# pythoncrazy/jimm

Hardware: AMD Instinct MI355X
Metric: images/sec (whole node) ViT-B/16@224 train (higher is better)
Workload: dtype bf16; 1 GPU; model=ViT-B/16@224, global_batch=1024, img_size=224, parallelism=dp1

## Files before the change

jimm_amd/csrc/gemm.hip:

```cpp

#include <torch/extension.h>
#include <ATen/hip/HIPContext.h>

#include "common.h"

namespace {

typedef short bf16x8_t __attribute__((ext_vector_type(8)));
typedef float f32x4_t __attribute__((ext_vector_type(4)));

#define MFMA16(A, B, C) __builtin_amdgcn_mfma_f32_16x16x32_bf16(A, B, C, 0, 0, 0)

constexpr int BM = 128, BN = 128, BK = 64;
constexpr int PITCH = BK + 8;



__device__ __forceinline__ void stage_tile_glds(const bf16* __restrict__ gsrc, int64_t ldg,
                                                short* lds_base, int tid) {
  const int wave = tid / WAVE;
  const int lane = tid % WAVE;
#pragma unroll
  for (int round = 0; round < 4; ++round) {
    const int off = round * 4096 + wave * 1024 + lane * 16;
    const int row = off >> 7;
    const int chunk = (off >> 4) & 7;
    const int src_chunk = chunk ^ (row & 7);
    const bf16* g = gsrc + (int64_t)row * ldg + src_chunk * 8;
    typedef const __attribute__((address_space(1))) unsigned int* gp_t;
    typedef __attribute__((address_space(3))) unsigned int* lp_t;
    __builtin_amdgcn_global_load_lds((gp_t)(const void*)g,
                                     (lp_t)(void*)(reinterpret_cast<char*>(lds_base) + round * 4096 + wave * 1024),
                                     16, 0, 0);
  }
}

__device__ __forceinline__ bf16x8_t lds_read_frag(const short* base, int row, int chunk) {
  const int byte = (row << 7) + ((chunk ^ (row & 7)) << 4);
  return *reinterpret_cast<const bf16x8_t*>(reinterpret_cast<const char*>(base) + byte);
}

template <int ACT, bool HAS_BIAS, bool HAS_RES, bool SAVE_PRE>
__global__ __launch_bounds__(256) void gemm_nt_fast_kernel(
    const bf16* __restrict__ X, const bf16* __restrict__ W, const float* __restrict__ bias,
    const bf16* __restrict__ res, bf16* __restrict__ Y, bf16* __restrict__ Z,
    int M, int N, int K) {
  extern __shared__ __attribute__((aligned(16))) char smem[];
  short* smem_s = reinterpret_cast<short*>(smem);
  auto xs = [&](int buf) { return smem_s + buf * 8192; };
  auto ws = [&](int buf) { return smem_s + 16384 + buf * 8192; };

  const int tid = threadIdx.x;
  const int lane = tid % WAVE;
  const int wave = tid / WAVE;
  const int lo = lane & 15, hi = lane >> 4;

  const int mt = M / BM, nt = N / BN;
  const int nwg = mt * nt;
  int wg = blockIdx.x;
  {
    const int q = nwg / 8, r = nwg % 8;
    const int xcd = wg % 8, idx = wg / 8;
    wg = (xcd < r ? xcd * (q + 1) : r * (q + 1) + (xcd - r) * q) + idx;
  }
  const int m0 = (wg / nt) * BM;
  const int n0 = (wg % nt) * BN;
  const int wm = (wave >> 1) * 64, wn = (wave & 1) * 64;

  f32x4_t acc[4][4] = {};

  stage_tile_glds(X + (int64_t)m0 * K, K, xs(0), tid);
  stage_tile_glds(W + (int64_t)n0 * K, K, ws(0), tid);
  __syncthreads();

  const int nk = K / BK;
  for (int kt = 0; kt < nk; ++kt) {
    const int buf = kt & 1;
    if (kt + 1 < nk) {
      stage_tile_glds(X + (int64_t)m0 * K + (kt + 1) * BK, K, xs(buf ^ 1), tid);
      stage_tile_glds(W + (int64_t)n0 * K + (kt + 1) * BK, K, ws(buf ^ 1), tid);
    }
#pragma unroll
    for (int ks = 0; ks < 2; ++ks) {
      bf16x8_t xa[4], wb[4];
#pragma unroll
      for (int mi = 0; mi < 4; ++mi) xa[mi] = lds_read_frag(xs(buf), wm + 16 * mi + lo, 4 * ks + hi);
#pragma unroll
      for (int ni = 0; ni < 4; ++ni) wb[ni] = lds_read_frag(ws(buf), wn + 16 * ni + lo, 4 * ks + hi);
#pragma unroll
      for (int mi = 0; mi < 4; ++mi)
#pragma unroll
        for (int ni = 0; ni < 4; ++ni) acc[mi][ni] = MFMA16(xa[mi], wb[ni], acc[mi][ni]);
    }
    __syncthreads();
  }

#pragma unroll
  for (int mi = 0; mi < 4; ++mi) {
#pragma unroll
    for (int r = 0; r < 4; ++r) {
      const int m = m0 + wm + 16 * mi + hi * 4 + r;
#pragma unroll
      for (int ni = 0; ni < 4; ++ni) {
        const int n = n0 + wn + 16 * ni + lo;
        float vpre = acc[mi][ni][r];
        if (HAS_BIAS) vpre += bias[n];
        if (SAVE_PRE) Z[(int64_t)m * N + n] = f2bf(vpre);
        float vy = act_fwd(vpre, ACT);
        if (HAS_RES) vy += bf2f(res[(int64_t)m * N + n]);
        Y[(int64_t)m * N + n] = f2bf(vy);
      }
    }
  }
}


template <int ACT, bool HAS_BIAS, bool HAS_RES, bool SAVE_PRE>
__global__ __launch_bounds__(256) void gemm_nt_kernel(
    const bf16* __restrict__ X, const bf16* __restrict__ W, const float* __restrict__ bias,
    const bf16* __restrict__ res, bf16* __restrict__ Y, bf16* __restrict__ Z,
    int M, int N, int K) {
  extern __shared__ __attribute__((aligned(16))) char smem[];
  short* xs = reinterpret_cast<short*>(smem);
  short* ws = xs + 2 * BM * PITCH;

  const int tid = threadIdx.x;
  const int wave = tid / WAVE;
  const int lane = tid % WAVE;
  const int lo = lane & 15, hi = lane >> 4;

  const int m0 = blockIdx.x * BM;
  const int n0 = blockIdx.y * BN;
  const int wm = (wave >> 1) * 64;
  const int wn = (wave & 1) * 64;

  f32x4_t acc[4][4] = {};

  auto stage = [&](int buf, int k0) {
    short* xd = xs + buf * BM * PITCH;
    short* wd = ws + buf * BN * PITCH;
    const int row = tid / 2;
    const int c0 = (tid & 1) * 32;
#pragma unroll
    for (int h = 0; h < 2; ++h) {
      const int cc = c0 + h * 16;
      if (m0 + row < M) {
        *reinterpret_cast<bf16x8_t*>(xd + row * PITCH + cc) =
            *reinterpret_cast<const bf16x8_t*>(X + (int64_t)(m0 + row) * K + k0 + cc);
        *reinterpret_cast<bf16x8_t*>(xd + row * PITCH + cc + 8) =
            *reinterpret_cast<const bf16x8_t*>(X + (int64_t)(m0 + row) * K + k0 + cc + 8);
      } else {
        for (int i = 0; i < 16; ++i) xd[row * PITCH + cc + i] = 0;
      }
      if (n0 + row < N) {
        *reinterpret_cast<bf16x8_t*>(wd + row * PITCH + cc) =
            *reinterpret_cast<const bf16x8_t*>(W + (int64_t)(n0 + row) * K + k0 + cc);
        *reinterpret_cast<bf16x8_t*>(wd + row * PITCH + cc + 8) =
            *reinterpret_cast<const bf16x8_t*>(W + (int64_t)(n0 + row) * K + k0 + cc + 8);
      } else {
        for (int i = 0; i < 16; ++i) wd[row * PITCH + cc + i] = 0;
      }
    }
  };

  stage(0, 0);
  __syncthreads();

  const int nk = K / BK;
  for (int kt = 0; kt < nk; ++kt) {
    const int buf = kt & 1;
    if (kt + 1 < nk) stage(buf ^ 1, (kt + 1) * BK);
    short* xd = xs + buf * BM * PITCH;
    short* wd = ws + buf * BN * PITCH;
#pragma unroll
    for (int ks = 0; ks < 2; ++ks) {
      bf16x8_t xa[4], wb[4];
#pragma unroll
      for (int mi = 0; mi < 4; ++mi)
        xa[mi] = *reinterpret_cast<const bf16x8_t*>(xd + (wm + 16 * mi + lo) * PITCH + 32 * ks + hi * 8);
#pragma unroll
      for (int ni = 0; ni < 4; ++ni)
        wb[ni] = *reinterpret_cast<const bf16x8_t*>(wd + (wn + 16 * ni + lo) * PITCH + 32 * ks + hi * 8);
#pragma unroll
      for (int mi = 0; mi < 4; ++mi)
#pragma unroll
        for (int ni = 0; ni < 4; ++ni)
          acc[mi][ni] = MFMA16(xa[mi], wb[ni], acc[mi][ni]);
    }
    __syncthreads();
  }

#pragma unroll
  for (int mi = 0; mi < 4; ++mi) {
#pragma unroll
    for (int r = 0; r < 4; ++r) {
      const int m = m0 + wm + 16 * mi + hi * 4 + r;
      if (m >= M) continue;
#pragma unroll
      for (int ni = 0; ni < 4; ++ni) {
        const int n = n0 + wn + 16 * ni + lo;
        if (n >= N) continue;
        float vpre = acc[mi][ni][r];
        if (HAS_BIAS) vpre += bias[n];
        if (SAVE_PRE) Z[(int64_t)m * N + n] = f2bf(vpre);
        float vy = act_fwd(vpre, ACT);
        if (HAS_RES) vy += bf2f(res[(int64_t)m * N + n]);
        Y[(int64_t)m * N + n] = f2bf(vy);
      }
    }
  }
}

}

bool gemm256_supported(int64_t M, int64_t N, int64_t K);
void gemm_nt_256(torch::Tensor x, torch::Tensor w, c10::optional<torch::Tensor> bias_f32,
                 std::string act, c10::optional<torch::Tensor> residual, torch::Tensor y,
                 c10::optional<torch::Tensor> z);
bool gemm8p_supported(int64_t M, int64_t N, int64_t K);
void gemm_nt_8p(torch::Tensor x, torch::Tensor w, c10::optional<torch::Tensor> bias_f32,
                std::string act, c10::optional<torch::Tensor> residual, torch::Tensor y,
                c10::optional<torch::Tensor> z);

static int gemm_tile_mode() {
  const char* env = getenv("JIMM_AMD_GEMM_TILE");
  if (!env) return 0;
  return atoi(env);
}

bool gemm_supported(int64_t M, int64_t N, int64_t K, std::string dtype) {
  if (dtype != "torch.bfloat16") return false;
  if (K % BK != 0) return false;
  const char* env = getenv("JIMM_AMD_GEMM");
  if (env && std::string(env) == "blas") return false;
  return true;
}

std::vector<torch::Tensor> linear_fwd(torch::Tensor x, torch::Tensor w,
                                      c10::optional<torch::Tensor> bias, std::string act,
                                      c10::optional<torch::Tensor> residual, bool save_z) {
  TORCH_CHECK(x.is_cuda() && x.is_contiguous() && w.is_contiguous());
  TORCH_CHECK(x.scalar_type() == torch::kBFloat16 && w.scalar_type() == torch::kBFloat16);
  const int M = x.size(0), K = x.size(1), N = w.size(0);
  TORCH_CHECK(w.size(1) == K && K % BK == 0);
  auto y = torch::empty({M, N}, x.options());
  torch::Tensor z;
  if (save_z) z = torch::empty({M, N}, x.options());
  c10::optional<torch::Tensor> bf;
  if (bias) bf = bias->contiguous().to(torch::kFloat32);
  int act_code = ACT_NONE;
  if (act == "gelu") act_code = ACT_GELU;
  else if (act == "gelu_tanh") act_code = ACT_GELU_TANH;
  else if (act == "quickgelu") act_code = ACT_QUICKGELU;
  else TORCH_CHECK(act.empty(), "unknown act ", act);

  const int tile_mode = gemm_tile_mode();
  if (tile_mode == 0 && gemm8p_supported(M, N, K)) {
    c10::optional<torch::Tensor> zopt;
    if (save_z) zopt = z;
    gemm_nt_8p(x, w, bf, act, residual, y, zopt);
    if (save_z) return {y, z};
    return {y, torch::Tensor()};
  }
  if (tile_mode != 128 && gemm256_supported(M, N, K)) {
    c10::optional<torch::Tensor> zopt;
    if (save_z) zopt = z;
    gemm_nt_256(x, w, bf, act, residual, y, zopt);
    if (save_z) return {y, z};
    return {y, torch::Tensor()};
  }

  auto stream = at::hip::getCurrentHIPStream();
  const bf16* resp = residual ? reinterpret_cast<const bf16*>(residual->data_ptr()) : nullptr;
  const float* biasp = bf ? bf->data_ptr<float>() : nullptr;
  bf16* zp = save_z ? reinterpret_cast<bf16*>(z.data_ptr()) : nullptr;
  const bool fast = (M % BM == 0) && (N % BN == 0);

#define LAUNCH(ACTC, HB, HR, SP)                                                          \
  do {                                                                                    \
    if (fast) {                                                                           \
      hipLaunchKernelGGL((gemm_nt_fast_kernel<ACTC, HB, HR, SP>),                         \
                         dim3((M / BM) * (N / BN)), dim3(256), 4 * 8192 * sizeof(short),  \
                         stream, reinterpret_cast<const bf16*>(x.data_ptr()),             \
                         reinterpret_cast<const bf16*>(w.data_ptr()), biasp, resp,        \
                         reinterpret_cast<bf16*>(y.data_ptr()), zp, M, N, K);             \
    } else {                                                                              \
      hipLaunchKernelGGL((gemm_nt_kernel<ACTC, HB, HR, SP>),                              \
                         dim3((M + BM - 1) / BM, (N + BN - 1) / BN), dim3(256),           \
                         2 * (BM + BN) * PITCH * sizeof(short), stream,                   \
                         reinterpret_cast<const bf16*>(x.data_ptr()),                     \
                         reinterpret_cast<const bf16*>(w.data_ptr()), biasp, resp,        \
                         reinterpret_cast<bf16*>(y.data_ptr()), zp, M, N, K);             \
    }                                                                                     \
  } while (0)
#define DISPATCH_ACT(HB, HR, SP)                                                          \
  switch (act_code) {                                                                     \
    case ACT_NONE: LAUNCH(ACT_NONE, HB, HR, SP); break;                                   \
    case ACT_GELU: LAUNCH(ACT_GELU, HB, HR, SP); break;                                   \
    case ACT_GELU_TANH: LAUNCH(ACT_GELU_TANH, HB, HR, SP); break;                         \
    case ACT_QUICKGELU: LAUNCH(ACT_QUICKGELU, HB, HR, SP); break;                         \
  }
  const bool hb = bias.has_value(), hr = residual.has_value();
  if (hb && hr && save_z) DISPATCH_ACT(true, true, true)
  else if (hb && hr) DISPATCH_ACT(true, true, false)
  else if (hb && save_z) DISPATCH_ACT(true, false, true)
  else if (hb) DISPATCH_ACT(true, false, false)
  else if (hr && save_z) DISPATCH_ACT(false, true, true)
  else if (hr) DISPATCH_ACT(false, true, false)
  else if (save_z) DISPATCH_ACT(false, false, true)
  else DISPATCH_ACT(false, false, false)
#undef DISPATCH_ACT
#undef LAUNCH
  if (save_z) return {y, z};
  return {y, torch::Tensor()};
}
```

jimm_amd/csrc/gemm8p.hip:

```cpp

#include <torch/extension.h>
#include <hip/hip_fp8.h>
#include <ATen/hip/HIPContext.h>

#include "common.h"

namespace {

typedef short bf16x8_t __attribute__((ext_vector_type(8)));
typedef float f32x4_t __attribute__((ext_vector_type(4)));

#define MFMA16(A, B, C) __builtin_amdgcn_mfma_f32_16x16x32_bf16(A, B, C, 0, 0, 0)

constexpr int BM = 256, BN = 256, BK = 64;
constexpr int NTHREADS = 512;
constexpr int HALF_BYTES = 128 * BK * 2;

__device__ __forceinline__ void raw_barrier() {
  asm volatile("s_barrier" ::: "memory");
}

template <bool MGUARD>
__device__ __forceinline__ const bf16* stage_base(const bf16* __restrict__ gsrc,
                                                  int64_t ldg, int row0, int rows_total,
                                                  int round, int tid) {
  const int off = round * 8192 + tid * 16;
  const int row = off >> 7;
  const int chunk = ((off >> 4) & 7) ^ (row & 7);
  int grow = row0 + row;
  if (MGUARD) grow = grow < rows_total ? grow : rows_total - 1;
  return gsrc + (int64_t)grow * ldg + chunk * 8;
}

__device__ __forceinline__ void glds16(const bf16* g, char* lds_dst) {
  typedef const __attribute__((address_space(1))) unsigned int* gp_t;
  typedef __attribute__((address_space(3))) unsigned int* lp_t;
  __builtin_amdgcn_global_load_lds((gp_t)(const void*)g, (lp_t)(void*)lds_dst, 16, 0, 0);
}

__device__ __forceinline__ bf16x8_t lds_frag8p(const char* base, int byte_off) {
  return *reinterpret_cast<const bf16x8_t*>(base + byte_off);
}

__device__ __forceinline__ int frag_off(int row, int chunk) {
  return (row << 7) + ((chunk ^ (row & 7)) << 4);
}

template <int ACT, bool HAS_BIAS, bool HAS_RES, bool SAVE_PRE, bool MGUARD, bool GRADM = false,
          bool FP8O = false>
__global__ __launch_bounds__(NTHREADS, 2) void gemm_nt_8p_kernel(
    const bf16* __restrict__ X, const bf16* __restrict__ W, const float* __restrict__ bias,
    const bf16* __restrict__ res, bf16* __restrict__ Y, bf16* __restrict__ Z,
    int M, int N, int K, unsigned char* __restrict__ Y8 = nullptr,
    const float* __restrict__ scale8 = nullptr,
    unsigned int* __restrict__ amax_bits = nullptr) {
  extern __shared__ __attribute__((aligned(16))) char smem[];
  auto As = [&](int buf, int h) { return smem + (buf * 2 + h) * HALF_BYTES; };
  auto Bs = [&](int slot, int h) {
    return smem + 4 * HALF_BYTES + (slot * 2 + h) * HALF_BYTES;
  };

  const int tid = threadIdx.x;
  const int lane = tid % WAVE;
  const int wave = tid / WAVE;
  const int lo = lane & 15, hi = lane >> 4;

  const int mt = MGUARD ? (M + BM - 1) / BM : M / BM;
  const int nt = N / BN;
  const int nwg = mt * nt;
  int wg = blockIdx.x;
  {
    const int q = nwg / 8, r = nwg % 8;
    const int xcd = wg % 8, idx = wg / 8;
    wg = (xcd < r ? xcd * (q + 1) : r * (q + 1) + (xcd - r) * q) + idx;
  }
  const int m0 = (wg / nt) * BM;
  const int n0 = (wg % nt) * BN;
  const int wm = (wave >> 2);
  const int wn = (wave & 3);

  f32x4_t acc[2][4][4] = {};

  const int nk = K / BK;
  const bf16* asrc[2][2];
  const bf16* bsrc[2][2];
#pragma unroll
  for (int h = 0; h < 2; ++h)
#pragma unroll
    for (int r = 0; r < 2; ++r) {
      asrc[h][r] = stage_base<MGUARD>(X, K, m0 + h * 128, M, r, tid);
      bsrc[h][r] = stage_base<false>(W + (int64_t)n0 * K, K, h * 128, N, r, tid);
    }
  const int ldst = tid * 16;
  auto stageA = [&](int kt, int h) {
    char* img = As(kt & 1, h);
    glds16(asrc[h][0] + (int64_t)kt * BK, img + ldst);
    glds16(asrc[h][1] + (int64_t)kt * BK, img + 8192 + ldst);
  };
  auto stageB = [&](int kt, int slot, int h) {
    char* img = Bs(slot, h);
    glds16(bsrc[h][0] + (int64_t)kt * BK, img + ldst);
    glds16(bsrc[h][1] + (int64_t)kt * BK, img + 8192 + ldst);
  };

  int offA[2][4], offB[2][4];
#pragma unroll
  for (int kh = 0; kh < 2; ++kh) {
#pragma unroll
    for (int mi = 0; mi < 4; ++mi)
      offA[kh][mi] = frag_off(wm * 64 + 16 * mi + lo, 4 * kh + hi);
#pragma unroll
    for (int ni = 0; ni < 4; ++ni)
      offB[kh][ni] = frag_off((wn & 1) * 64 + 16 * ni + lo, 4 * kh + hi);
  }
  const int bh = wn >> 1;

  stageB(0, 0, 0);
  stageB(0, 0, 1);
  stageA(0, 0);
  stageA(0, 1);
  asm volatile("s_waitcnt vmcnt(2)" ::: "memory");
  raw_barrier();

  int slot = 0, slot1 = nk > 1 ? 1 : 0;
  for (int t = 0; t < nk; ++t) {
    const int buf = t & 1;
    const char* a0i = As(buf, 0);
    const char* a1i = As(buf, 1);
    const char* bi = Bs(slot, bh);
    const bool more = t + 1 < nk;
#pragma unroll
    for (int kh = 0; kh < 2; ++kh) {
      bf16x8_t xa[4], wb[4];
#pragma unroll
      for (int mi = 0; mi < 4; ++mi) xa[mi] = lds_frag8p(a0i, offA[kh][mi]);
#pragma unroll
      for (int ni = 0; ni < 4; ++ni) wb[ni] = lds_frag8p(bi, offB[kh][ni]);
      if (more) {
        if (kh == 0) stageB(t + 1, slot1, 0);
        else stageA(t + 1, 0);
      }
      if (kh == 0) {
        if (t == nk - 1) asm volatile("s_waitcnt vmcnt(0)" ::: "memory");
        else asm volatile("s_waitcnt vmcnt(2)" ::: "memory");
      } else {
        asm volatile("s_waitcnt vmcnt(4)" ::: "memory");
      }
      raw_barrier();
      __builtin_amdgcn_s_setprio(1);
#pragma unroll
      for (int mi = 0; mi < 4; ++mi)
#pragma unroll
        for (int ni = 0; ni < 4; ++ni)
          acc[0][mi][ni] = MFMA16(xa[mi], wb[ni], acc[0][mi][ni]);
      __builtin_amdgcn_s_setprio(0);

#pragma unroll
      for (int mi = 0; mi < 4; ++mi) xa[mi] = lds_frag8p(a1i, offA[kh][mi]);
      if (more) {
        if (kh == 0) stageB(t + 1, slot1, 1);
        else stageA(t + 1, 1);
      }
      if (kh == 0) asm volatile("s_waitcnt vmcnt(4)" ::: "memory");
      else asm volatile("s_waitcnt vmcnt(2)" ::: "memory");
      raw_barrier();
      __builtin_amdgcn_s_setprio(1);
#pragma unroll
      for (int mi = 0; mi < 4; ++mi)
#pragma unroll
        for (int ni = 0; ni < 4; ++ni)
          acc[1][mi][ni] = MFMA16(xa[mi], wb[ni], acc[1][mi][ni]);
      __builtin_amdgcn_s_setprio(0);
    }
    slot = slot1;
    slot1 = slot1 + 1 == 3 ? 0 : slot1 + 1;
  }

  float rs8 = 1.f, tmax = 0.f;
  if (FP8O) rs8 = 1.f / scale8[0];
#pragma unroll
  for (int pr = 0; pr < 2; ++pr) {
#pragma unroll
    for (int mi = 0; mi < 4; ++mi) {
#pragma unroll
      for (int r = 0; r < 4; ++r) {
        const int m = m0 + pr * 128 + wm * 64 + 16 * mi + hi * 4 + r;
        if (MGUARD && m >= M) continue;
#pragma unroll
        for (int ni = 0; ni < 4; ++ni) {
          const int n = n0 + wn * 64 + 16 * ni + lo;
          float vpre = acc[pr][mi][ni][r];
          if (HAS_BIAS) vpre += bias[n];
          if (SAVE_PRE) Z[(int64_t)m * N + n] = f2bf(vpre);
          float vy;
          if (GRADM) {
            vy = vpre * act_grad(bf2f(res[(int64_t)m * N + n]), ACT);
          } else {
            vy = act_fwd(vpre, ACT);
            if (HAS_RES) vy += bf2f(res[(int64_t)m * N + n]);
          }
          Y[(int64_t)m * N + n] = f2bf(vy);
          if (FP8O) {
            tmax = fmaxf(tmax, fabsf(vy));
            Y8[(int64_t)m * N + n] = cvt_e4m3(vy * rs8);
          }
        }
      }
    }
  }
  if (FP8O) {
    tmax = wave_reduce_max(tmax);
    if (lane == 0) atomicMax(amax_bits, __float_as_uint(tmax));
  }
}

}

bool gemm8p_supported(int64_t M, int64_t N, int64_t K) {
  return M >= 1 && (N % BN == 0) && (K % BK == 0) && K >= 2 * BK;
}

torch::Tensor gemm_nt_8p_gradact(torch::Tensor dy, torch::Tensor wt, torch::Tensor z,
                                 std::string act) {
  const int M = dy.size(0), K = dy.size(1), N = wt.size(0);
  TORCH_CHECK(dy.is_contiguous() && wt.is_contiguous() && z.is_contiguous());
  TORCH_CHECK(wt.size(1) == K && z.size(0) == M && z.size(1) == N);
  TORCH_CHECK(gemm8p_supported(M, N, K));
  int act_code = ACT_NONE;
  if (act == "gelu") act_code = ACT_GELU;
  else if (act == "gelu_tanh") act_code = ACT_GELU_TANH;
  else if (act == "quickgelu") act_code = ACT_QUICKGELU;
  else TORCH_CHECK(false, "gradact needs an activation, got ", act);
  auto y = torch::empty({M, N}, dy.options());
  auto stream = at::hip::getCurrentHIPStream();
  const size_t shmem = 10 * HALF_BYTES;
  const bool mguard = (M % BM) != 0;
  const int mt = (M + BM - 1) / BM;
#define LAUNCH_GRAD(ACTC, MG)                                                              \
  do {                                                                                     \
    auto kfn = gemm_nt_8p_kernel<ACTC, false, true, false, MG, true>;                      \
    static bool attr_g_##ACTC##MG = [&] {                                                  \
      hipFuncSetAttribute(reinterpret_cast<const void*>(kfn),                              \
                          hipFuncAttributeMaxDynamicSharedMemorySize, (int)shmem);         \
      return true;                                                                         \
    }();                                                                                   \
    (void)attr_g_##ACTC##MG;                                                               \
    hipLaunchKernelGGL(kfn, dim3(mt * (N / BN)), dim3(NTHREADS), shmem, stream,            \
                       reinterpret_cast<const bf16*>(dy.data_ptr()),                       \
                       reinterpret_cast<const bf16*>(wt.data_ptr()), nullptr,              \
                       reinterpret_cast<const bf16*>(z.data_ptr()),                        \
                       reinterpret_cast<bf16*>(y.data_ptr()), nullptr, M, N, K,            \
                       nullptr, nullptr, nullptr);                                         \
  } while (0)
#define DG(ACTC)                                                                           \
  do {                                                                                     \
    if (mguard) LAUNCH_GRAD(ACTC, true);                                                   \
    else LAUNCH_GRAD(ACTC, false);                                                         \
  } while (0)
  switch (act_code) {
    case ACT_GELU: DG(ACT_GELU); break;
    case ACT_GELU_TANH: DG(ACT_GELU_TANH); break;
    case ACT_QUICKGELU: DG(ACT_QUICKGELU); break;
  }
#undef DG
#undef LAUNCH_GRAD
  return y;
}

std::vector<torch::Tensor> gemm_nt_8p_gradact_fp8(torch::Tensor dy, torch::Tensor wt,
                                                  torch::Tensor z, std::string act,
                                                  torch::Tensor scale8, torch::Tensor amax) {
  const int M = dy.size(0), K = dy.size(1), N = wt.size(0);
  TORCH_CHECK(dy.is_contiguous() && wt.is_contiguous() && z.is_contiguous());
  TORCH_CHECK(wt.size(1) == K && z.size(0) == M && z.size(1) == N);
  TORCH_CHECK(gemm8p_supported(M, N, K));
  int act_code = ACT_NONE;
  if (act == "gelu") act_code = ACT_GELU;
  else if (act == "gelu_tanh") act_code = ACT_GELU_TANH;
  else if (act == "quickgelu") act_code = ACT_QUICKGELU;
  else TORCH_CHECK(false, "gradact needs an activation, got ", act);
  auto y = torch::empty({M, N}, dy.options());
  auto y8 = torch::empty({M, N}, dy.options().dtype(torch::kUInt8));
  auto stream = at::hip::getCurrentHIPStream();
  const size_t shmem = 10 * HALF_BYTES;
  const bool mguard = (M % BM) != 0;
  const int mt = (M + BM - 1) / BM;
#define LAUNCH_GRAD8(ACTC, MG)                                                             \
  do {                                                                                     \
    auto kfn = gemm_nt_8p_kernel<ACTC, false, true, false, MG, true, true>;                \
    static bool attr_g8_##ACTC##MG = [&] {                                                 \
      hipFuncSetAttribute(reinterpret_cast<const void*>(kfn),                              \
                          hipFuncAttributeMaxDynamicSharedMemorySize, (int)shmem);         \
      return true;                                                                         \
    }();                                                                                   \
    (void)attr_g8_##ACTC##MG;                                                              \
    hipLaunchKernelGGL(kfn, dim3(mt * (N / BN)), dim3(NTHREADS), shmem, stream,            \
                       reinterpret_cast<const bf16*>(dy.data_ptr()),                       \
                       reinterpret_cast<const bf16*>(wt.data_ptr()), nullptr,              \
                       reinterpret_cast<const bf16*>(z.data_ptr()),                        \
                       reinterpret_cast<bf16*>(y.data_ptr()), nullptr, M, N, K,            \
                       y8.data_ptr<unsigned char>(), scale8.data_ptr<float>(),             \
                       reinterpret_cast<unsigned int*>(amax.data_ptr()));                  \
  } while (0)
#define DG8(ACTC)                                                                          \
  do {                                                                                     \
    if (mguard) LAUNCH_GRAD8(ACTC, true);                                                  \
    else LAUNCH_GRAD8(ACTC, false);                                                        \
  } while (0)
  switch (act_code) {
    case ACT_GELU: DG8(ACT_GELU); break;
    case ACT_GELU_TANH: DG8(ACT_GELU_TANH); break;
    case ACT_QUICKGELU: DG8(ACT_QUICKGELU); break;
  }
#undef DG8
#undef LAUNCH_GRAD8
  return {y, y8};
}

void gemm_nt_8p(torch::Tensor x, torch::Tensor w, c10::optional<torch::Tensor> bias_f32,
                std::string act, c10::optional<torch::Tensor> residual, torch::Tensor y,
                c10::optional<torch::Tensor> z) {
  const int M = x.size(0), K = x.size(1), N = w.size(0);
  TORCH_CHECK(gemm8p_supported(M, N, K));
  int act_code = ACT_NONE;
  if (act == "gelu") act_code = ACT_GELU;
  else if (act == "gelu_tanh") act_code = ACT_GELU_TANH;
  else if (act == "quickgelu") act_code = ACT_QUICKGELU;
  else TORCH_CHECK(act.empty(), "unknown act ", act);
  auto stream = at::hip::getCurrentHIPStream();
  const bf16* resp = residual ? reinterpret_cast<const bf16*>(residual->data_ptr()) : nullptr;
  const float* biasp = bias_f32 ? bias_f32->data_ptr<float>() : nullptr;
  bf16* zp = z ? reinterpret_cast<bf16*>(z->data_ptr()) : nullptr;
  const size_t shmem = 10 * HALF_BYTES;
  const bool mguard = (M % BM) != 0;
  const int mt = (M + BM - 1) / BM;

#define LAUNCH8P(ACTC, HB, HR, SP, MG)                                                     \
  do {                                                                                     \
    auto kfn = gemm_nt_8p_kernel<ACTC, HB, HR, SP, MG>;                                    \
    static bool attr_set_##ACTC##HB##HR##SP##MG = [&] {                                    \
      hipFuncSetAttribute(reinterpret_cast<const void*>(kfn),                              \
                          hipFuncAttributeMaxDynamicSharedMemorySize, (int)shmem);         \
      return true;                                                                         \
    }();                                                                                   \
    (void)attr_set_##ACTC##HB##HR##SP##MG;                                                 \
    hipLaunchKernelGGL(kfn, dim3(mt * (N / BN)), dim3(NTHREADS), shmem, stream,            \
                       reinterpret_cast<const bf16*>(x.data_ptr()),                        \
                       reinterpret_cast<const bf16*>(w.data_ptr()), biasp, resp,           \
                       reinterpret_cast<bf16*>(y.data_ptr()), zp, M, N, K,                 \
                       nullptr, nullptr, nullptr);                                         \
  } while (0)
#define DISPATCH_MG(ACTC, HB, HR, SP)                                                      \
  do {                                                                                     \
    if (mguard) LAUNCH8P(ACTC, HB, HR, SP, true);                                          \
    else LAUNCH8P(ACTC, HB, HR, SP, false);                                                \
  } while (0)
#define DISPATCH_ACT8P(HB, HR, SP)                                                         \
  switch (act_code) {                                                                      \
    case ACT_NONE: DISPATCH_MG(ACT_NONE, HB, HR, SP); break;                               \
    case ACT_GELU: DISPATCH_MG(ACT_GELU, HB, HR, SP); break;                               \
    case ACT_GELU_TANH: DISPATCH_MG(ACT_GELU_TANH, HB, HR, SP); break;                     \
    case ACT_QUICKGELU: DISPATCH_MG(ACT_QUICKGELU, HB, HR, SP); break;                     \
  }
  const bool hb = bias_f32.has_value(), hr = residual.has_value(), sp = z.has_value();
  if (hb && hr && sp) DISPATCH_ACT8P(true, true, true)
  else if (hb && hr) DISPATCH_ACT8P(true, true, false)
  else if (hb && sp) DISPATCH_ACT8P(true, false, true)
  else if (hb) DISPATCH_ACT8P(true, false, false)
  else if (hr && sp) DISPATCH_ACT8P(false, true, true)
  else if (hr) DISPATCH_ACT8P(false, true, false)
  else if (sp) DISPATCH_ACT8P(false, false, true)
  else DISPATCH_ACT8P(false, false, false)
#undef DISPATCH_ACT8P
#undef DISPATCH_MG
#undef LAUNCH8P
}
```

Before: 5808 images/sec.

## Transpose MFMA operands and permute W rows for vectorized GEMM epilogue stores

Swaps the MFMA operand order so each lane holds 16 contiguous output columns per row, with a matching row permutation when staging the W tile so those columns line up. The epilogue then uses 16-byte vector loads and stores for bias, residual, Z, Y and the FP8 output in place of scalar per-element accesses. It also drops the per-call conversion of the bias to fp32 on the 8p path by reading bf16 bias directly. The cost is extra alignment checks and clones, and the permuted layout makes correctness more subtle.

```diff
diff --git a/jimm_amd/csrc/gemm.hip b/jimm_amd/csrc/gemm.hip
--- a/jimm_amd/csrc/gemm.hip
+++ b/jimm_amd/csrc/gemm.hip
@@ -218,7 +218,7 @@
                  std::string act, c10::optional<torch::Tensor> residual, torch::Tensor y,
                  c10::optional<torch::Tensor> z);
 bool gemm8p_supported(int64_t M, int64_t N, int64_t K);
-void gemm_nt_8p(torch::Tensor x, torch::Tensor w, c10::optional<torch::Tensor> bias_f32,
+void gemm_nt_8p(torch::Tensor x, torch::Tensor w, c10::optional<torch::Tensor> bias,
                 std::string act, c10::optional<torch::Tensor> residual, torch::Tensor y,
                 c10::optional<torch::Tensor> z);
 
@@ -246,8 +246,6 @@
   auto y = torch::empty({M, N}, x.options());
   torch::Tensor z;
   if (save_z) z = torch::empty({M, N}, x.options());
-  c10::optional<torch::Tensor> bf;
-  if (bias) bf = bias->contiguous().to(torch::kFloat32);
   int act_code = ACT_NONE;
   if (act == "gelu") act_code = ACT_GELU;
   else if (act == "gelu_tanh") act_code = ACT_GELU_TANH;
@@ -258,10 +256,14 @@
   if (tile_mode == 0 && gemm8p_supported(M, N, K)) {
     c10::optional<torch::Tensor> zopt;
     if (save_z) zopt = z;
-    gemm_nt_8p(x, w, bf, act, residual, y, zopt);
+    c10::optional<torch::Tensor> b8 = bias;
+    if (bias && bias->scalar_type() != torch::kBFloat16) b8 = bias->to(torch::kFloat32);
+    gemm_nt_8p(x, w, b8, act, residual, y, zopt);
     if (save_z) return {y, z};
     return {y, torch::Tensor()};
   }
+  c10::optional<torch::Tensor> bf;
+  if (bias) bf = bias->contiguous().to(torch::kFloat32);
   if (tile_mode != 128 && gemm256_supported(M, N, K)) {
     c10::optional<torch::Tensor> zopt;
     if (save_z) zopt = z;
diff --git a/jimm_amd/csrc/gemm8p.hip b/jimm_amd/csrc/gemm8p.hip
--- a/jimm_amd/csrc/gemm8p.hip
+++ b/jimm_amd/csrc/gemm8p.hip
@@ -20,14 +20,16 @@
   asm volatile("s_barrier" ::: "memory");
 }
 
-template <bool MGUARD>
+template <bool MGUARD, bool PERM = false>
 __device__ __forceinline__ const bf16* stage_base(const bf16* __restrict__ gsrc,
                                                   int64_t ldg, int row0, int rows_total,
                                                   int round, int tid) {
   const int off = round * 8192 + tid * 16;
   const int row = off >> 7;
   const int chunk = ((off >> 4) & 7) ^ (row & 7);
-  int grow = row0 + row;
+  int srow = row;
+  if (PERM) srow = (row & 64) | ((row & 12) << 2) | ((row >> 2) & 12) | (row & 3);
+  int grow = row0 + srow;
   if (MGUARD) grow = grow < rows_total ? grow : rows_total - 1;
   return gsrc + (int64_t)grow * ldg + chunk * 8;
 }
@@ -49,8 +51,8 @@
 template <int ACT, bool HAS_BIAS, bool HAS_RES, bool SAVE_PRE, bool MGUARD, bool GRADM = false,
           bool FP8O = false>
 __global__ __launch_bounds__(NTHREADS, 2) void gemm_nt_8p_kernel(
-    const bf16* __restrict__ X, const bf16* __restrict__ W, const float* __restrict__ bias,
-    const bf16* __restrict__ res, bf16* __restrict__ Y, bf16* __restrict__ Z,
+    const bf16* __restrict__ X, const bf16* __restrict__ W, const void* __restrict__ bias,
+    int bias_is_f32, const bf16* __restrict__ res, bf16* __restrict__ Y, bf16* __restrict__ Z,
     int M, int N, int K, unsigned char* __restrict__ Y8 = nullptr,
     const float* __restrict__ scale8 = nullptr,
     unsigned int* __restrict__ amax_bits = nullptr) {
@@ -89,7 +91,7 @@
 #pragma unroll
     for (int r = 0; r < 2; ++r) {
       asrc[h][r] = stage_base<MGUARD>(X, K, m0 + h * 128, M, r, tid);
-      bsrc[h][r] = stage_base<false>(W + (int64_t)n0 * K, K, h * 128, N, r, tid);
+      bsrc[h][r] = stage_base<false, true>(W + (int64_t)n0 * K, K, h * 128, N, r, tid);
     }
   const int ldst = tid * 16;
   auto stageA = [&](int kt, int h) {
@@ -152,7 +154,7 @@
       for (int mi = 0; mi < 4; ++mi)
 #pragma unroll
         for (int ni = 0; ni < 4; ++ni)
-          acc[0][mi][ni] = MFMA16(xa[mi], wb[ni], acc[0][mi][ni]);
+          acc[0][mi][ni] = MFMA16(wb[ni], xa[mi], acc[0][mi][ni]);
       __builtin_amdgcn_s_setprio(0);
 
 #pragma unroll
@@ -169,42 +171,86 @@
       for (int mi = 0; mi < 4; ++mi)
 #pragma unroll
         for (int ni = 0; ni < 4; ++ni)
-          acc[1][mi][ni] = MFMA16(xa[mi], wb[ni], acc[1][mi][ni]);
+          acc[1][mi][ni] = MFMA16(wb[ni], xa[mi], acc[1][mi][ni]);
       __builtin_amdgcn_s_setprio(0);
     }
     slot = slot1;
     slot1 = slot1 + 1 == 3 ? 0 : slot1 + 1;
   }
 
+  const int nb = n0 + wn * 64 + hi * 16;
+  float bv[16];
+  if (HAS_BIAS) {
+    if (bias_is_f32) {
+      const float* bp = reinterpret_cast<const float*>(bias) + nb;
+#pragma unroll
+      for (int q = 0; q < 4; ++q) {
+        float t[4];
+        vload_f32<4>(bp + 4 * q, t);
+#pragma unroll
+        for (int j = 0; j < 4; ++j) bv[4 * q + j] = t[j];
+      }
+    } else {
+      const bf16* bp = reinterpret_cast<const bf16*>(bias) + nb;
+#pragma unroll
+      for (int q = 0; q < 2; ++q) {
+        float t[8];
+        vload_f32<8>(bp + 8 * q, t);
+#pragma unroll
+        for (int j = 0; j < 8; ++j) bv[8 * q + j] = t[j];
+      }
+    }
+  }
   float rs8 = 1.f, tmax = 0.f;
   if (FP8O) rs8 = 1.f / scale8[0];
 #pragma unroll
   for (int pr = 0; pr < 2; ++pr) {
 #pragma unroll
     for (int mi = 0; mi < 4; ++mi) {
-#pragma unroll
-      for (int r = 0; r < 4; ++r) {
-        const int m = m0 + pr * 128 + wm * 64 + 16 * mi + hi * 4 + r;
-        if (MGUARD && m >= M) continue;
-#pragma unroll
-        for (int ni = 0; ni < 4; ++ni) {
-          const int n = n0 + wn * 64 + 16 * ni + lo;
+      const int m = m0 + pr * 128 + wm * 64 + 16 * mi + lo;
+      if (MGUARD && m >= M) continue;
+      const int64_t o = (int64_t)m * N + nb;
+      float rv[2][8];
+      if (HAS_RES || GRADM) {
+        vload_f32<8>(res + o, rv[0]);
+        vload_f32<8>(res + o + 8, rv[1]);
+      }
+      float vz[2][8], vo[2][8];
+#pragma unroll
+      for (int ni = 0; ni < 4; ++ni) {
+#pragma unroll
+        for (int r = 0; r < 4; ++r) {
+          const int j = 4 * ni + r;
           float vpre = acc[pr][mi][ni][r];
-          if (HAS_BIAS) vpre += bias[n];
-          if (SAVE_PRE) Z[(int64_t)m * N + n] = f2bf(vpre);
+          if (HAS_BIAS) vpre += bv[j];
+          vz[j >> 3][j & 7] = vpre;
           float vy;
           if (GRADM) {
-            vy = vpre * act_grad(bf2f(res[(int64_t)m * N + n]), ACT);
+            vy = vpre * act_grad(rv[j >> 3][j & 7], ACT);
           } else {
             vy = act_fwd(vpre, ACT);
-            if (HAS_RES) vy += bf2f(res[(int64_t)m * N + n]);
+            if (HAS_RES) vy += rv[j >> 3][j & 7];
           }
-          Y[(int64_t)m * N + n] = f2bf(vy);
-          if (FP8O) {
-            tmax = fmaxf(tmax, fabsf(vy));
-            Y8[(int64_t)m * N + n] = cvt_e4m3(vy * rs8);
-          }
+          vo[j >> 3][j & 7] = vy;
         }
+      }
+      if (SAVE_PRE) {
+        vstore_f32<8>(Z + o, vz[0]);
+        vstore_f32<8>(Z + o + 8, vz[1]);
+      }
+      vstore_f32<8>(Y + o, vo[0]);
+      vstore_f32<8>(Y + o + 8, vo[1]);
+      if (FP8O) {
+        unsigned int pk[4];
+#pragma unroll
+        for (int q = 0; q < 4; ++q) {
+          const float* v4 = &vo[q >> 1][(q & 1) * 4];
+#pragma unroll
+          for (int j = 0; j < 4; ++j) tmax = fmaxf(tmax, fabsf(v4[j]));
+          pk[q] = (unsigned int)cvt2_e4m3(v4[0] * rs8, v4[1] * rs8) |
+                  ((unsigned int)cvt2_e4m3(v4[2] * rs8, v4[3] * rs8) << 16);
+        }
+        *reinterpret_cast<uint4*>(Y8 + o) = make_uint4(pk[0], pk[1], pk[2], pk[3]);
       }
     }
   }
@@ -218,6 +264,12 @@
 
 bool gemm8p_supported(int64_t M, int64_t N, int64_t K) {
   return M >= 1 && (N % BN == 0) && (K % BK == 0) && K >= 2 * BK;
+}
+
+static torch::Tensor aligned16(const torch::Tensor& t) {
+  auto c = t.contiguous();
+  if (reinterpret_cast<uintptr_t>(c.data_ptr()) % 16 != 0) c = c.clone();
+  return c;
 }
 
 torch::Tensor gemm_nt_8p_gradact(torch::Tensor dy, torch::Tensor wt, torch::Tensor z,
@@ -226,6 +278,7 @@
   TORCH_CHECK(dy.is_contiguous() && wt.is_contiguous() && z.is_contiguous());
   TORCH_CHECK(wt.size(1) == K && z.size(0) == M && z.size(1) == N);
   TORCH_CHECK(gemm8p_supported(M, N, K));
+  z = aligned16(z);
   int act_code = ACT_NONE;
   if (act == "gelu") act_code = ACT_GELU;
   else if (act == "gelu_tanh") act_code = ACT_GELU_TANH;
@@ -247,7 +300,7 @@
     (void)attr_g_##ACTC##MG;                                                               \
     hipLaunchKernelGGL(kfn, dim3(mt * (N / BN)), dim3(NTHREADS), shmem, stream,            \
                        reinterpret_cast<const bf16*>(dy.data_ptr()),                       \
-                       reinterpret_cast<const bf16*>(wt.data_ptr()), nullptr,              \
+                       reinterpret_cast<const bf16*>(wt.data_ptr()), nullptr, 0,           \
                        reinterpret_cast<const bf16*>(z.data_ptr()),                        \
                        reinterpret_cast<bf16*>(y.data_ptr()), nullptr, M, N, K,            \
                        nullptr, nullptr, nullptr);                                         \
@@ -274,6 +327,7 @@
   TORCH_CHECK(dy.is_contiguous() && wt.is_contiguous() && z.is_contiguous());
   TORCH_CHECK(wt.size(1) == K && z.size(0) == M && z.size(1) == N);
   TORCH_CHECK(gemm8p_supported(M, N, K));
+  z = aligned16(z);
   int act_code = ACT_NONE;
   if (act == "gelu") act_code = ACT_GELU;
   else if (act == "gelu_tanh") act_code = ACT_GELU_TANH;
@@ -296,7 +350,7 @@
     (void)attr_g8_##ACTC##MG;                                                              \
     hipLaunchKernelGGL(kfn, dim3(mt * (N / BN)), dim3(NTHREADS), shmem, stream,            \
                        reinterpret_cast<const bf16*>(dy.data_ptr()),                       \
-                       reinterpret_cast<const bf16*>(wt.data_ptr()), nullptr,              \
+                       reinterpret_cast<const bf16*>(wt.data_ptr()), nullptr, 0,           \
                        reinterpret_cast<const bf16*>(z.data_ptr()),                        \
                        reinterpret_cast<bf16*>(y.data_ptr()), nullptr, M, N, K,            \
                        y8.data_ptr<unsigned char>(), scale8.data_ptr<float>(),             \
@@ -317,11 +371,24 @@
   return {y, y8};
 }
 
-void gemm_nt_8p(torch::Tensor x, torch::Tensor w, c10::optional<torch::Tensor> bias_f32,
+void gemm_nt_8p(torch::Tensor x, torch::Tensor w, c10::optional<torch::Tensor> bias,
                 std::string act, c10::optional<torch::Tensor> residual, torch::Tensor y,
                 c10::optional<torch::Tensor> z) {
   const int M = x.size(0), K = x.size(1), N = w.size(0);
   TORCH_CHECK(gemm8p_supported(M, N, K));
+  if (bias) {
+    TORCH_CHECK(bias->scalar_type() == torch::kBFloat16 ||
+                    bias->scalar_type() == torch::kFloat32,
+                "gemm_nt_8p: bias must be bf16 or fp32");
+    TORCH_CHECK(bias->numel() == N);
+    bias = aligned16(*bias);
+  }
+  if (residual) {
+    TORCH_CHECK(residual->scalar_type() == torch::kBFloat16 && residual->numel() == (int64_t)M * N);
+    residual = aligned16(*residual);
+  }
+  TORCH_CHECK(reinterpret_cast<uintptr_t>(y.data_ptr()) % 16 == 0 &&
+              (!z || reinterpret_cast<uintptr_t>(z->data_ptr()) % 16 == 0));
   int act_code = ACT_NONE;
   if (act == "gelu") act_code = ACT_GELU;
   else if (act == "gelu_tanh") act_code = ACT_GELU_TANH;
@@ -329,7 +396,8 @@
   else TORCH_CHECK(act.empty(), "unknown act ", act);
   auto stream = at::hip::getCurrentHIPStream();
   const bf16* resp = residual ? reinterpret_cast<const bf16*>(residual->data_ptr()) : nullptr;
-  const float* biasp = bias_f32 ? bias_f32->data_ptr<float>() : nullptr;
+  const void* biasp = bias ? bias->data_ptr() : nullptr;
+  const int bias_f32 = bias && bias->scalar_type() == torch::kFloat32;
   bf16* zp = z ? reinterpret_cast<bf16*>(z->data_ptr()) : nullptr;
   const size_t shmem = 10 * HALF_BYTES;
   const bool mguard = (M % BM) != 0;
@@ -346,7 +414,7 @@
     (void)attr_set_##ACTC##HB##HR##SP##MG;                                                 \
     hipLaunchKernelGGL(kfn, dim3(mt * (N / BN)), dim3(NTHREADS), shmem, stream,            \
                        reinterpret_cast<const bf16*>(x.data_ptr()),                        \
-                       reinterpret_cast<const bf16*>(w.data_ptr()), biasp, resp,           \
+                       reinterpret_cast<const bf16*>(w.data_ptr()), biasp, bias_f32, resp, \
                        reinterpret_cast<bf16*>(y.data_ptr()), zp, M, N, K,                 \
                        nullptr, nullptr, nullptr);                                         \
   } while (0)
@@ -362,7 +430,7 @@
     case ACT_GELU_TANH: DISPATCH_MG(ACT_GELU_TANH, HB, HR, SP); break;                     \
     case ACT_QUICKGELU: DISPATCH_MG(ACT_QUICKGELU, HB, HR, SP); break;                     \
   }
-  const bool hb = bias_f32.has_value(), hr = residual.has_value(), sp = z.has_value();
+  const bool hb = bias.has_value(), hr = residual.has_value(), sp = z.has_value();
   if (hb && hr && sp) DISPATCH_ACT8P(true, true, true)
   else if (hb && hr) DISPATCH_ACT8P(true, true, false)
   else if (hb && sp) DISPATCH_ACT8P(true, false, true)
```

Measured after the change: 5860 images/sec (median of 6 runs). No clear change (+0.9%).
